# quantumjot/sequitr

Measured on AMD Instinct MI355X. Metric: segmented Mpixels/sec on 512x512 tiles; IoU vs reference, higher is better.
Workload: dtype f32; 1 GPU; U-Net 2-class inference, launches of 32 512x512x1 tiles, fp32 (BASELINE.json configs[1]: filters 16-32-64-128-256, eltwise_mul bridge); logits + uint8 argmax mask; one 32-tile batch per GPU per step; tiles_this_rank=32

## Files before the change

### include/sequitr_hip.h

```cpp
#ifndef SEQUITR_HIP_H
#define SEQUITR_HIP_H

#include <stdint.h>

#ifdef __cplusplus
extern "C" {
#endif

#define SQ_OK 0
#define SQ_EINVAL (-1)
#define SQ_ELAUNCH (-2)
#define SQ_EALIGN (-3)

#define SQ_ACT_NONE 0
#define SQ_ACT_RELU 1
#define SQ_ACT_LEAKY 2

#define SQ_BRIDGE_NONE 0
#define SQ_BRIDGE_ADD 1
#define SQ_BRIDGE_MUL 2
#define SQ_BRIDGE_SUB 3

int sq_version(void);
const char *sq_last_error(void);
// ... 104 lines not shown
int sq_scale_f32(const float *x, float *y, int64_t n, int64_t per_sample, float s, const float *s_per_sample,
                 int one_minus, void *stream);

int sq_act_fwd_f32(const float *x, float *y, int64_t n, int act, void *stream);

int64_t sq_dot_per_sample_workspace_f32(int N);
int sq_dot_per_sample_f32(const float *a, const float *b, float *out, float *workspace, int N, int64_t per_sample,
                          void *stream);

int sq_mbstd_fwd_f32(const float *x, float *out, float *workspace, int N, int64_t per_sample, void *stream);
int64_t sq_mbstd_map_workspace(int groups);
int sq_mbstd_map_fwd_f32(const float *x, float *y, float *workspace, int groups, int n, int64_t per_sample, int cells,
                         void *stream);
int sq_mbstd_map_bwd_f32(const float *x, const float *dy, float *dx, float *workspace, int groups, int n,
                         int64_t per_sample, int cells, void *stream);
int sq_mbstd_map_bwd2_f32(const float *x, const float *dy, const float *v, float *ddy, float *dx2, float *workspace,
                          int groups, int n, int64_t per_sample, int cells, void *stream);
int sq_mbstd_map_fwd_bf16(const void *x, float *y, float *workspace, int groups, int n, int64_t per_sample, int cells, void *stream);
int sq_mbstd_map_bwd_bf16(const void *x, const float *dy, void *dx, float *workspace, int groups, int n, int64_t per_sample,
                          int cells, void *stream);
int sq_mbstd_map_bwd2_bf16(const void *x, const float *dy, const void *v, float *ddy, void *dx2, float *workspace, int groups,
                           int n, int64_t per_sample, int cells, void *stream);
int sq_wgan_losses_fwd_f32(const float *Dz, const float *Dx, const float *gn2, float *out2, int N, void *stream);
int sq_wgan_losses_bwd_f32(const float *Dz, const float *Dx, const float *gn2, const float *g_dloss, const float *g_gloss,
                           float *dDz, float *dDx, float *dgn2, int N, void *stream);

int sq_mosaic_pack_f32(const float *x, float *m, int N, int H, int W, int C, int R, int Cc, void *stream);
int sq_mosaic_unpack_f32(const float *m, float *y, int N, int H, int W, int C, int R, int Cc, void *stream);

int64_t sq_dense_workspace_f32(int M, int K, int N);
int sq_dense_fwd_f32(const float *x, const float *w, const float *bias, float *y, float *workspace, int M, int K, int N,
                     float wscale, int act, void *stream);
int sq_dense_wgrad_f32(const float *x, const float *dy, float *dw, float *db, int M, int K, int N, float scale, int accumulate,
                       void *stream);

int64_t sq_wgrad1x1_small_workspace_f32(int64_t npix, int Ca, int Cb);
int sq_wgrad1x1_small_f32(const float *a, const float *b, float *m, float *workspace, int64_t npix, int Ca, int Cb,
                          void *stream);


int sq_conv2d_concat_nhwc_fwd_f32(const float *xa, const float *xb, const float *w, const float *bias, float *y, int N,
                                  int H, int W, int Ca, int Cout, int K, int act, void *stream);

int sq_conv3x3_pool_fwd_f32(const float *x, const float *w, const float *bias, float *y, float *pooled,
                            int N, int H, int W, int Cin, int Cout, int act, void *stream);

int64_t sq_conv_packed_filter_elems_f32(int K, int Cin, int Cout);
int sq_conv_pack_filter_f32(const float *w, float *wp, int K, int Cin, int Cout, void *stream);
int sq_conv_packed_takes_f32(int N, int H, int W, int Cin, int Cout, int K);
int sq_conv2d_packed_nhwc_fwd_f32(const float *x, const float *w, const float *wp, const float *bias, float *y, int N, int H,
                                  int W, int Cin, int Cout, int K, float wscale, int act, void *stream);
int sq_conv3x3_pool_packed_fwd_f32(const float *x, const float *w, const float *wp, const float *bias, float *y, float *pooled,
                                   int N, int H, int W, int Cin, int Cout, int act, void *stream);

int sq_conv_r32_takes_f32(int N, int H, int W, int Cin, int Cout, int K, int act, int pooled);

int sq_conv3x3_head_fwd_f32(const float *x, const float *w, const float *bias, const float *head_w,
                            const float *head_b, float *logits, uint8_t *mask, int N, int H, int W,
                            int Cin, int head_c, int act, void *stream);

int sq_conv3x3_first_block_fwd_f32(const float *x, const float *w1, const float *b1, const float *w2,
                                   const float *b2, float *y, float *pooled, int N, int H, int W,
                                   void *stream);

int sq_convT_conv3x3_fwd_f32(const float *x_low, const float *wt, const float *bt, const float *skip, int bridge,
                             const float *w, const float *bias, float *y, int N, int H, int W, int act, void *stream);


int64_t sq_conv_packed_weights_elems_bf16(int K, int Cin, int Cout);
int sq_conv_pack_weights_bf16(const float *w, void *wp, int K, int Cin, int Cout, float wscale, int transform,
                              void *stream);
int sq_conv_pack_weights_multi_bf16(const float *base, void *out, const int32_t *table, int n_entries,
                                    int total_items, void *stream);
int sq_conv_pack_weights_multi_scaled_bf16(const float *base, void *out, const int32_t *table, const float *scales,
                                           int n_entries, int total_items, void *stream);

int sq_conv2d_nhwc_fwd_bf16(const void *x, const void *wp, const float *bias, void *y, int N, int H, int W,
                            int Cin, int Cout, int K, int act, void *stream);

int sq_conv2d_nhwc_fwd_mixed_f32(const float *x, const void *wp, const float *bias, float *y, int N, int H, int W,
                                 int Cin, int Cout, int K, int act, void *stream);
int sq_conv2d_nhwc_dgrad_actgate_mixed_f32(const float *dy, const void *wp_t, const float *gate, int act, float *dx, int N,
                                           int H, int W, int Cin, int Cout, int K, void *stream);
int sq_conv2d_nhwc_mixed_mosaic_f32(const float *x, const void *wp, const float *bias, const float *gate, float *y, int Nimg,
                                    int h, int w, int Cin, int Cout, int act, int R, int Cc, void *stream);
int64_t sq_conv2d_nhwc_wgrad_workspace_mixed_f32(int N, int H, int W, int Cin, int Cout, int K);
int sq_conv2d_nhwc_wgrad_mixed_f32(const float *x, const float *dy, float *dw, float *db, float *workspace, int N,
                                   int H, int W, int Cin, int Cout, int K, void *stream);
int sq_conv2d_nhwc_wgrad_scaled_mixed_f32(const float *x, const float *dy, float *dw, float *db, float *workspace, int N,
                                          int H, int W, int Cin, int Cout, int K, float dw_scale, void *stream);
int sq_conv2d_nhwc_wgrad_mixed_mosaic_f32(const float *x, const float *dy, float *dw, float *db, float *workspace, int Nimg,
                                          int h, int w, int Cin, int Cout, int R, int Cc, float dw_scale, void *stream);
int sq_conv2d_nhwc_wgrad_scaled_f32(const float *x, const float *dy, float *dw, float *db, float *workspace, int N, int H,
                                    int W, int Cin, int Cout, int K, float dw_scale, void *stream);

int sq_conv3x3_first_fwd_bf16(const float *x, const float *w, const float *bias, void *y, int N, int H, int W,
                              int Cin, int Cout, int act, void *stream);
int sq_conv3x3_first_fwd_mask_bf16(const float *x, const float *w, const float *bias, void *y, void *mask, int N, int H,
                                   int W, int Cin, int Cout, int act, void *stream);
int sq_conv2d_nhwc_fwd_mask_bf16(const void *x, const void *wp, const float *bias, void *y, void *mask, int N, int H, int W,
                                 int Cin, int Cout, int K, int act, void *stream);
int sq_conv2d_nhwc_dgrad_maskgate_bf16(const void *dy, const void *wp_t, const void *mask, float scale, void *dx, int N,
                                       int H, int W, int Cin, int Cout, int K, void *stream);

int64_t sq_conv2d_nhwc_wgrad_workspace_bf16(int N, int H, int W, int Cin, int Cout, int K);
int sq_conv2d_nhwc_wgrad_bf16(const void *x, const void *dy, float *dw, float *db, float *workspace, int N,
// ... 399 lines not shown
```

### sequitr_amd/_lib.py

```python
import ctypes
import os

_HERE = os.path.dirname(os.path.abspath(__file__))
LIB_PATH = os.path.join(_HERE, "_build", "libsequitr_hip.so")

c_void_p, c_int, c_float, c_int64 = ctypes.c_void_p, ctypes.c_int, ctypes.c_float, ctypes.c_int64


class WgradItem(ctypes.Structure):
    _fields_ = [("x", c_void_p), ("dy", c_void_p), ("dw", c_void_p), ("db", c_void_p),
                ("N", ctypes.c_int32), ("H", ctypes.c_int32), ("W", ctypes.c_int32), ("Cin", ctypes.c_int32),
                ("Cout", ctypes.c_int32), ("K", ctypes.c_int32), ("convT_cout", ctypes.c_int32), ("dw_scale", c_float),
                ("accumulate", ctypes.c_int32), ("mosaic_R", ctypes.c_int32), ("mosaic_Cc", ctypes.c_int32),
                ("reserved", ctypes.c_int32)]

SIGNATURES = {
    "sq_version": (c_int, []),
    "sq_last_error": (ctypes.c_char_p, []),
    "sq_conv2d_nhwc_fwd_f32": (c_int, [c_void_p] * 4 + [c_int] * 6 + [c_float, c_int, c_void_p]),
    "sq_maxpool2x2_fwd_f32": (c_int, [c_void_p] * 2 + [c_int] * 4 + [c_void_p]),
    "sq_avgpool2x2_fwd_f32": (c_int, [c_void_p] * 2 + [c_int] * 4 + [c_void_p]),
    "sq_convT2x2s2_nhwc_fwd_f32": (c_int, [c_void_p] * 5 + [c_int] * 6 + [c_void_p]),
    "sq_bridge_fwd_f32": (c_int, [c_void_p] * 3 + [c_int64, c_int, c_void_p]),
    "sq_conv1x1_argmax_fwd_f32": (c_int, [c_void_p] * 5 + [c_int] * 5 + [c_void_p]),
# ... 102 lines not shown
    "sq_convT_conv3x3_fwd_f32": (c_int, [c_void_p] * 4 + [c_int] + [c_void_p] * 3 + [c_int] * 4 + [c_void_p]),
    "sq_volume_centroids_u8": (c_int, [c_void_p, c_int, c_int, c_int, c_int, c_void_p, c_void_p, c_void_p, c_void_p, c_int,
                                       c_void_p]),
    "sq_mosaic_pack_f32": (c_int, [c_void_p, c_void_p] + [c_int] * 6 + [c_void_p]),
    "sq_mosaic_unpack_f32": (c_int, [c_void_p, c_void_p] + [c_int] * 6 + [c_void_p]),
    "sq_zero_insert2x_f32": (c_int, [c_void_p, c_void_p, c_int, c_int, c_int, c_int, c_void_p]),
    "sq_gather_odd2x_f32": (c_int, [c_void_p, c_void_p, c_int, c_int, c_int, c_int, c_void_p]),
    "sq_bn_workspace_f32": (c_int64, [c_int64, c_int]),
    "sq_bn_stats_f32": (c_int, [c_void_p] * 4 + [c_int64, c_int, c_void_p]),
    "sq_bn_stats_bf16": (c_int, [c_void_p] * 4 + [c_int64, c_int, c_void_p]),
    "sq_bn_fold_f32": (c_int, [c_void_p] * 4 + [c_float, c_void_p, c_void_p, c_int, c_void_p]),
    "sq_bn_update_moving_f32": (c_int, [c_void_p] * 4 + [c_float, c_int64, c_int, c_void_p]),
    "sq_bn_apply_f32": (c_int, [c_void_p] * 4 + [c_int64, c_int, c_int, c_void_p]),
    "sq_bn_apply_bf16": (c_int, [c_void_p] * 4 + [c_int64, c_int, c_int, c_void_p]),
    "sq_bn_bwd_f32": (c_int, [c_void_p] * 3 + [c_int] + [c_void_p] * 3 + [c_float] + [c_void_p] * 4
                      + [c_int64, c_int, c_void_p]),
    "sq_bn_bwd_bf16": (c_int, [c_void_p] * 3 + [c_int] + [c_void_p] * 3 + [c_float] + [c_void_p] * 4
                      + [c_int64, c_int, c_void_p]),
    "sq_adam_step_dev_f32": (c_int, [c_void_p] * 4 + [c_int64] + [c_float] * 4 + [c_void_p, c_float, c_void_p]),
    "sq_adam_advance_dev": (c_int, [c_void_p, c_float, c_float, c_float, c_void_p]),
    "sq_adam_advance_warmup_dev": (c_int, [c_void_p, c_float, c_float, c_float, c_int, c_void_p]),
    "sq_adam_apply_dev_f32": (c_int, [c_void_p] * 4 + [c_int64, c_float, c_float, c_float, c_void_p, c_float, c_void_p]),
    "sq_adam_multi_chunk": (c_int, []),
    "sq_adam_apply_multi_dev_f32": (c_int, [c_void_p, c_int, c_int64, c_float, c_float, c_float, c_void_p, c_float, c_void_p]),
    "sq_pixelnorm_bwd_f32": (c_int, [c_void_p] * 3 + [c_int64, c_int, c_float, c_void_p]),
    "sq_pixelnorm_bwd2_f32": (c_int, [c_void_p] * 5 + [c_int64, c_int, c_float, c_void_p]),
    "sq_pixelnorm_bwd_act_f32": (c_int, [c_void_p] * 3 + [c_int64, c_int, c_float, c_int, c_void_p]),
    "sq_broadcast2x2_act_bwd_f32": (c_int, [c_void_p] * 3 + [c_int] * 4 + [c_float, c_int, c_void_p]),
    "sq_resize_nearest_f32": (c_int, [c_void_p] * 2 + [c_int] * 6 + [c_void_p]),
    "sq_lerp_f32": (c_int, [c_void_p] * 3 + [c_int64, c_int64, c_float, c_void_p, c_void_p]),
    "sq_scale_f32": (c_int, [c_void_p] * 2 + [c_int64, c_int64, c_float, c_void_p, c_int, c_void_p]),
    "sq_act_fwd_f32": (c_int, [c_void_p] * 2 + [c_int64, c_int, c_void_p]),
    "sq_dot_per_sample_workspace_f32": (c_int64, [c_int]),
    "sq_dot_per_sample_f32": (c_int, [c_void_p] * 4 + [c_int, c_int64, c_void_p]),
    "sq_mbstd_fwd_f32": (c_int, [c_void_p] * 3 + [c_int, c_int64, c_void_p]),
    "sq_mbstd_map_workspace": (c_int64, [c_int]),
    "sq_mbstd_map_fwd_f32": (c_int, [c_void_p] * 3 + [c_int, c_int, c_int64, c_int, c_void_p]),
    "sq_mbstd_map_bwd_f32": (c_int, [c_void_p] * 4 + [c_int, c_int, c_int64, c_int, c_void_p]),
    "sq_mbstd_map_bwd2_f32": (c_int, [c_void_p] * 6 + [c_int, c_int, c_int64, c_int, c_void_p]),
    "sq_mbstd_map_fwd_bf16": (c_int, [c_void_p] * 3 + [c_int, c_int, c_int64, c_int, c_void_p]),
    "sq_mbstd_map_bwd_bf16": (c_int, [c_void_p] * 4 + [c_int, c_int, c_int64, c_int, c_void_p]),
    "sq_mbstd_map_bwd2_bf16": (c_int, [c_void_p] * 6 + [c_int, c_int, c_int64, c_int, c_void_p]),
    "sq_wgan_losses_fwd_f32": (c_int, [c_void_p] * 4 + [c_int, c_void_p]),
    "sq_wgan_losses_bwd_f32": (c_int, [c_void_p] * 8 + [c_int, c_void_p]),
    "sq_dense_wgrad_f32": (c_int, [c_void_p] * 4 + [c_int] * 3 + [c_float, c_int, c_void_p]),
    "sq_wgrad1x1_small_workspace_f32": (c_int64, [c_int64, c_int, c_int]),
    "sq_wgrad1x1_small_f32": (c_int, [c_void_p] * 4 + [c_int64, c_int, c_int, c_void_p]),
    "sq_conv2d_concat_nhwc_fwd_f32": (c_int, [c_void_p] * 5 + [c_int] * 7 + [c_void_p]),
    "sq_conv3x3_pool_fwd_f32": (c_int, [c_void_p] * 5 + [c_int] * 6 + [c_void_p]),
    "sq_conv3x3_head_fwd_f32": (c_int, [c_void_p] * 7 + [c_int] * 6 + [c_void_p]),
    "sq_conv_packed_filter_elems_f32": (c_int64, [c_int] * 3),
    "sq_conv_pack_filter_f32": (c_int, [c_void_p] * 2 + [c_int] * 3 + [c_void_p]),
    "sq_conv_packed_takes_f32": (c_int, [c_int] * 6),
    "sq_conv_r32_takes_f32": (c_int, [c_int] * 8),
    "sq_conv2d_packed_nhwc_fwd_f32": (c_int, [c_void_p] * 5 + [c_int] * 6 + [c_float, c_int, c_void_p]),
    "sq_conv3x3_pool_packed_fwd_f32": (c_int, [c_void_p] * 6 + [c_int] * 6 + [c_void_p]),
    "sq_conv3x3_first_block_fwd_f32": (c_int, [c_void_p] * 7 + [c_int] * 3 + [c_void_p]),
    "sq_conv_packed_weights_elems_bf16": (c_int64, [c_int] * 3),
    "sq_conv_pack_weights_bf16": (c_int, [c_void_p] * 2 + [c_int] * 3 + [c_float, c_int, c_void_p]),
    "sq_conv2d_nhwc_fwd_bf16": (c_int, [c_void_p] * 4 + [c_int] * 7 + [c_void_p]),
    "sq_conv2d_nhwc_fwd_mixed_f32": (c_int, [c_void_p] * 4 + [c_int] * 7 + [c_void_p]),
    "sq_conv2d_nhwc_wgrad_workspace_mixed_f32": (c_int64, [c_int] * 6),
    "sq_conv2d_nhwc_wgrad_mixed_f32": (c_int, [c_void_p] * 5 + [c_int] * 6 + [c_void_p]),
    "sq_conv2d_nhwc_wgrad_scaled_mixed_f32": (c_int, [c_void_p] * 5 + [c_int] * 6 + [c_float, c_void_p]),
    "sq_conv2d_nhwc_wgrad_scaled_f32": (c_int, [c_void_p] * 5 + [c_int] * 6 + [c_float, c_void_p]),
    "sq_conv3x3_first_fwd_bf16": (c_int, [c_void_p] * 4 + [c_int] * 6 + [c_void_p]),
    "sq_conv2d_nhwc_wgrad_workspace_bf16": (c_int64, [c_int] * 6),
    "sq_conv2d_nhwc_wgrad_bf16": (c_int, [c_void_p] * 5 + [c_int] * 6 + [c_void_p]),
    "sq_convT2x2s2_wgrad_bf16": (c_int, [c_void_p] * 5 + [c_int] * 5 + [c_void_p]),
    "sq_cast_f32_to_bf16": (c_int, [c_void_p] * 2 + [c_int64, c_void_p]),
    "sq_cast_bf16_to_f32": (c_int, [c_void_p] * 2 + [c_int64, c_void_p]),
    "sq_head_concat_fwd_bf16": (c_int, [c_void_p] * 3 + [c_int64, c_int, c_void_p]),
    "sq_head_concat_bwd_bf16": (c_int, [c_void_p] * 3 + [c_int64, c_int, c_void_p]),
    "sq_maxpool2x2_fwd_bf16": (c_int, [c_void_p] * 2 + [c_int] * 4 + [c_void_p]),
    "sq_maxpool2x2_bwd_bf16": (c_int, [c_void_p] * 3 + [c_int] * 4 + [c_void_p]),
    "sq_conv_pack_weights_multi_bf16": (c_int, [c_void_p, c_void_p, c_void_p, c_int, c_int, c_void_p]),
    "sq_conv_pack_weights_multi_scaled_bf16": (c_int, [c_void_p] * 4 + [c_int, c_int, c_void_p]),
    "sq_conv2d_nhwc_fwd_dropout_bf16": (c_int, [c_void_p] * 4 + [c_int] * 7 + [c_float, ctypes.c_uint32, c_void_p, c_void_p]),
    "sq_conv3x3_first_fwd_mask_bf16": (c_int, [c_void_p] * 5 + [c_int] * 6 + [c_void_p]),
    "sq_conv2d_nhwc_fwd_mask_bf16": (c_int, [c_void_p] * 5 + [c_int] * 7 + [c_void_p]),
    "sq_conv2d_nhwc_dgrad_maskgate_bf16": (c_int, [c_void_p] * 3 + [c_float, c_void_p] + [c_int] * 6 + [c_void_p]),
    "sq_conv2d_nhwc_wgrad_mixed_mosaic_f32": (c_int, [c_void_p] * 5 + [c_int] * 7 + [c_float, c_void_p]),
    "sq_conv2d_nhwc_mixed_mosaic_f32": (c_int, [c_void_p] * 5 + [c_int] * 8 + [c_void_p]),
    "sq_conv2d_nhwc_dgrad_actgate_mixed_f32": (c_int, [c_void_p] * 3 + [c_int, c_void_p] + [c_int] * 6 + [c_void_p]),
    "sq_conv2d_nhwc_fwd_dropout_pool_bf16": (c_int, [c_void_p] * 5 + [c_int] * 7 + [c_float, ctypes.c_uint32, c_void_p, c_void_p]),
    "sq_conv3x3_first_block_dropout_pool_bf16": (c_int, [c_void_p] * 9 + [c_int] * 3 + [c_float, ctypes.c_uint32, c_void_p, c_void_p]),
    "sq_relu_scale_bwd_bf16": (c_int, [c_void_p] * 3 + [c_int64, c_float, c_void_p]),
    "sq_bridge_bwd_s2d_bf16": (c_int, [c_void_p] * 5 + [c_int] * 5 + [c_void_p]),
    "sq_maxpool2x2_bwd_add_bf16": (c_int, [c_void_p] * 4 + [c_int] * 4 + [c_void_p]),
    "sq_maxpool2x2_bwd_add_gate_bf16": (c_int, [c_void_p] * 4 + [c_int] * 4 + [c_float, c_void_p]),
    "sq_conv2d_nhwc_dgrad_gate_bf16": (c_int, [c_void_p] * 3 + [c_float, c_void_p] + [c_int] * 6 + [c_void_p]),
    "sq_conv2d_nhwc_dgrad_junction_bf16": (c_int, [c_void_p] * 6 + [c_int] * 7 + [c_void_p]),
    "sq_conv1x1_head_bwd_gate_bf16": (c_int, [c_void_p] * 7 + [c_int64, c_int, c_int, c_float, c_void_p]),
    "sq_conv1x1_head_wce_fwd_bf16": (c_int, [c_void_p] * 7 + [c_int64, c_int, c_int, c_void_p]),
    "sq_conv1x1_head_wce_bwd_bf16": (c_int, [c_void_p] * 10 + [c_int64, c_int, c_int, c_float, c_void_p]),
    "sq_conv1x1_head_wce_bwd_loss_bf16": (c_int, [c_void_p] * 12 + [c_int64, c_int, c_int, c_float, c_void_p]),
    "sq_act_dropout_bwd_bf16": (c_int, [c_void_p] * 4 + [c_int64, c_float, c_int, c_void_p]),
    "sq_conv2d_nhwc_dgrad_relu_bf16": (c_int, [c_void_p] * 4 + [c_int] * 6 + [c_void_p]),
    "sq_pixelnorm_fwd_bf16": (c_int, [c_void_p] * 2 + [c_int64, c_int, c_float, c_void_p]),
    "sq_pixelnorm_bwd_bf16": (c_int, [c_void_p] * 3 + [c_int64, c_int, c_float, c_int, c_void_p]),
    "sq_pixelnorm_bwd2_bf16": (c_int, [c_void_p] * 5 + [c_int64, c_int, c_float, c_void_p]),
    "sq_sumpool2x2_bf16": (c_int, [c_void_p] * 2 + [c_int] * 4 + [c_float, c_void_p]),
    "sq_broadcast2x2_bf16": (c_int, [c_void_p] * 2 + [c_int] * 4 + [c_float, c_void_p]),
    "sq_broadcast2x2_act_bwd_bf16": (c_int, [c_void_p] * 3 + [c_int] * 4 + [c_float, c_int, c_void_p]),
    "sq_act_fwd_bf16": (c_int, [c_void_p] * 2 + [c_int64, c_int, c_void_p]),
    "sq_conv1x1_smallin_fwd_bf16": (c_int, [c_void_p] * 4 + [c_int64, c_int, c_int, c_float, c_int, c_void_p]),
# ... 72 lines not shown
```

### sequitr_amd/csrc/sq_conv_f32_packed.hip

```cpp
#include <stdlib.h>
#include <type_traits>
#include "sq_common.h"
#include "sq_conv_epi.h"

#ifndef SQ_PK_RING
#define SQ_PK_RING 4
#endif
#ifndef SQ_PK_OCC
#define SQ_PK_OCC 2
#endif
#ifndef SQ_PK_WRITE_AT
#define SQ_PK_WRITE_AT 22
#endif

namespace {

constexpr int TH = 16, TW = 16, BN = 64, KC = 16, NR = BN / 16;
constexpr int HALO_W = TW + 2, HALO_H = TH + 2, HP = HALO_W * HALO_H;
constexpr int PS = KC + 2;
constexpr int XS_FLOATS = HP * PS;
constexpr int QPP = KC / 4, XITEMS = HP * QPP, XSLOTS = (XITEMS + 255) / 256;
constexpr int NSTEP = 9 * (KC / 4);
constexpr int RING = SQ_PK_RING;
constexpr int STEP_BYTES = 64 * 16, ITEM_BYTES = NSTEP * STEP_BYTES;
constexpr int LDS_BYTES = (2 * XS_FLOATS + 64 * 4) * 4;
constexpr int OCC = SQ_PK_OCC;
static_assert(SQ_PK_OCC != 2 || sq_v2_occ(BN, KC, false) == 2, "the default walks the unpacked form's grid");
static_assert(NSTEP % RING == 0 && RING >= 2 && RING <= 6, "the ring slot of a step must not depend on the item");
static_assert(SQ_PK_WRITE_AT + XSLOTS <= NSTEP, "the halo writes must fit the item's steps");
static_assert((XS_FLOATS * 4) % 16 == 0, "second halo buffer must start 16-B aligned");

__global__ __launch_bounds__(256) void pack_filter_f32_kernel(const float *__restrict__ w, float4 *__restrict__ wp,
                                                              int Cin, int Cout, int total) {
    const int e = blockIdx.x * 256 + threadIdx.x;
    if (e >= total) return;
    const int lane = e & 63, li = lane & 15, kk = lane >> 4;
    int t = e >> 6;
    const int s = t & 3;
    t >>= 2;
    const int tap = t % 9;
    t /= 9;
    const int nchunk = Cin / KC, c = t % nchunk, cb = t / nchunk;
    const float *src = w + (size_t)(tap * Cin + c * KC + 4 * s + kk) * Cout + cb * BN + li;
    wp[e] = make_float4(src[0], src[16], src[32], src[48]);
}

__global__ __launch_bounds__(256, OCC) void conv_mfma_f32_packed_kernel(
    const float *__restrict__ x, const float *__restrict__ wp, const float *__restrict__ bias, float *__restrict__ y,
    int N, int H, int W, int Cin, int Cout, int act, int tiles_x, int tiles_y, int ntiles, float *__restrict__ pooled) {
    extern __shared__ __attribute__((aligned(16))) float smem[];
    const int tid = threadIdx.x, lane = tid & 63, wv = tid >> 6;
    __builtin_assume(tid < 256);
    const int li = lane & 15, kk = lane >> 4;
    const int n0 = blockIdx.y * BN;
    const int vb = (int)sq_xcd_remap(blockIdx.x, gridDim.x);
    const int tstride = (int)gridDim.x;
    const int t_begin = vb;
    if (t_begin >= ntiles) return;
    const int t_count = (ntiles - vb + tstride - 1) / tstride;
    const int nchunk = Cin / KC;
    const int nitems = t_count * nchunk;

    const __amdgpu_buffer_rsrc_t xrsrc = __builtin_amdgcn_make_buffer_rsrc(
        const_cast<float *>(x), 0, (int)((size_t)N * H * W * Cin * 4), 0x00020000);
    const __amdgpu_buffer_rsrc_t wrsrc = __builtin_amdgcn_make_buffer_rsrc(
        const_cast<float *>(wp), 0, 9 * Cin * Cout * 4, 0x00020000);
    const __amdgpu_buffer_rsrc_t yrsrc = __builtin_amdgcn_make_buffer_rsrc(y, 0, (int)((size_t)N * H * W * Cout * 4), 0x00020000);
    constexpr unsigned OOB = 0x80000000u;

    int xrel[XSLOTS], xpy[XSLOTS], xpx[XSLOTS];
#pragma unroll
    for (int sl = 0; sl < XSLOTS; ++sl) {
        const int idx = tid + sl * 256;
        const int pix = idx / QPP, q = idx % QPP;
        xpy[sl] = idx < XITEMS ? pix / HALO_W : (1 << 24);
        xpx[sl] = pix % HALO_W;
        xrel[sl] = idx < XITEMS ? ((pix / HALO_W * W + xpx[sl]) * Cin + q * 4) * 4 : (int)OOB;
    }
    float4 xr[XSLOTS];
    auto issue = [&](int tx, int ty, int n, int cc, bool live) {
        const int x0 = tx * TW - 1, y0 = ty * TH - 1;
        const int base = (((n * H + y0) * W + x0) * Cin + cc) * 4;
        const unsigned Hl = live ? (unsigned)H : 0u;
#pragma unroll
        for (int sl = 0; sl < XSLOTS; ++sl) {
            const bool inb = (unsigned)(y0 + xpy[sl]) < Hl && (unsigned)(x0 + xpx[sl]) < (unsigned)W;
            const unsigned off = inb ? (unsigned)(base + xrel[sl]) : OOB;
            const auto v = __builtin_amdgcn_raw_buffer_load_b128(xrsrc, off, 0, 0);
            xr[sl] = *reinterpret_cast<const float4 *>(&v);
        }
    };
    float *const dump = smem + 2 * XS_FLOATS + lane * 4;
    auto put_slot = [&](float *xs, int sl) {
        const int idx = tid + sl * 256;
        const int pix = idx / QPP, q = idx % QPP;
        float *d = idx < XITEMS ? xs + pix * PS + q * 4 : dump;
        *reinterpret_cast<float2 *>(d) = make_float2(xr[sl].x, xr[sl].y);
        *reinterpret_cast<float2 *>(d + 2) = make_float2(xr[sl].z, xr[sl].w);
    };

    const int a_lane = lane * 16;
    auto load_a = [&](int item_off, int st) {
        const auto v = __builtin_amdgcn_raw_buffer_load_b128(wrsrc, a_lane, item_off + st * STEP_BYTES, 0);
        return *reinterpret_cast<const float4 *>(&v);
    };
    const int xb_off = ((4 * wv) * HALO_W + li) * PS + kk;
    auto load_b = [&](const float *xs, int st, float (&b)[4]) {
        const int tap = st / 4, s = st % 4;
        const int ky = tap / 3, kx = tap % 3;
#pragma unroll
        for (int r = 0; r < 4; ++r) b[r] = xs[xb_off + ((r + ky) * HALO_W + kx) * PS + s * 4];
    };

    const float slope = act == SQ_ACT_LEAKY ? 0.2f : 1.0f;
    const bool is_relu = act == SQ_ACT_RELU;
    auto actk = [&](float v, auto fastc) {
        if constexpr (decltype(fastc)::value) return __builtin_fmaxf(v, 0.0f);
        else {
            const float neg = is_relu ? 0.0f : v * slope;
            return v > 0.0f ? v : neg;
        }
    };
    float4 bvr[NR];
#pragma unroll
    for (int nb = 0; nb < NR; ++nb)
        bvr[nb] = bias ? *reinterpret_cast<const float4 *>(bias + n0 + nb * 16 + 4 * kk) : make_float4(0.f, 0.f, 0.f, 0.f);
    const int fast_lane = (((4 * wv) * W + li) * Cout + 4 * kk) * 4;

    f32x4 acc[4][NR];
    auto epilogue = [&](int tx, int ty, int n, auto fastc) {
        constexpr bool FAST = decltype(fastc)::value;
        auto actf = [&](float v) { return actk(v, fastc); };
        const int gx = tx * TW + li;
#pragma unroll
        for (int nb = 0; nb < NR; ++nb) {
            const int co = n0 + nb * 16 + 4 * kk;
            const float4 bv = bvr[nb];
            f32x4 o[4];
#pragma unroll
            for (int r = 0; r < 4; ++r) {
                const int gy = ty * TH + 4 * wv + r;
                o[r][0] = actf(bias ? acc[r][nb][0] + bv.x : acc[r][nb][0]);
                o[r][1] = actf(bias ? acc[r][nb][1] + bv.y : acc[r][nb][1]);
                o[r][2] = actf(bias ? acc[r][nb][2] + bv.z : acc[r][nb][2]);
                o[r][3] = actf(bias ? acc[r][nb][3] + bv.w : acc[r][nb][3]);
                unsigned off;
                if constexpr (FAST) {
                    off = (unsigned)(fast_lane + nb * 64) + (unsigned)((((n * H + ty * TH + r) * W + tx * TW) * Cout + n0) * 4);
                } else {
                    const bool ok = gy < H && gx < W;
                    off = ok ? (unsigned)((((n * H + gy) * W + gx) * Cout + co) * 4) : OOB;
                }
                __builtin_amdgcn_raw_buffer_store_b128(
                    *reinterpret_cast<__attribute__((__vector_size__(4 * sizeof(unsigned)))) unsigned *>(&o[r]), yrsrc, off, 0, 0);
                acc[r][nb] = (f32x4){0.f, 0.f, 0.f, 0.f};
            }
            if (pooled) {
#pragma unroll
                for (int pr = 0; pr < 2; ++pr) {
                    float mp[4];
#pragma unroll
                    for (int j = 0; j < 4; ++j) {
                        const float a = o[2 * pr][j], b = o[2 * pr + 1][j];
                        const float v = b > a ? b : a;
                        const float u = __shfl_xor(v, 1);
                        mp[j] = u > v ? u : v;
                    }
                    const int py = (ty * TH + 4 * wv) / 2 + pr, px = gx >> 1;
                    if ((li & 1) == 0 && py < (H >> 1) && px < (W >> 1))
                        *reinterpret_cast<float4 *>(pooled + ((size_t)(n * (H >> 1) + py) * (W >> 1) + px) * Cout + co) =
                            make_float4(mp[0], mp[1], mp[2], mp[3]);
                }
            }
        }
    };

    const int per_image = tiles_x * tiles_y;
    const int s_n = tstride / per_image, s_y = (tstride % per_image) / tiles_x, s_x = (tstride % per_image) % tiles_x;
    int ctx = t_begin % tiles_x, cty = (t_begin / tiles_x) % tiles_y, cn = t_begin / per_image;
    int ntx = ctx + s_x, nty = cty, nn = cn;
    if (ntx >= tiles_x) { ntx -= tiles_x; nty += 1; }
    nty += s_y;
    if (nty >= tiles_y) { nty -= tiles_y; nn += 1; }
    nn += s_n;

    const int cb_off = blockIdx.y * nchunk * ITEM_BYTES;
    issue(ctx, cty, cn, 0, true);
    float4 ar[RING];
#pragma unroll
    for (int j = 0; j < RING; ++j) ar[j] = load_a(cb_off, j);
#pragma unroll
    for (int sl = 0; sl < XSLOTS; ++sl) put_slot(smem, sl);
#pragma unroll
    for (int r = 0; r < 4; ++r)
#pragma unroll
        for (int nb = 0; nb < NR; ++nb) acc[r][nb] = (f32x4){0.f, 0.f, 0.f, 0.f};
    __syncthreads();

    int chunk = 0;
    for (int it = 0; it < nitems; ++it) {
        const float *xs = smem + (it & 1) * XS_FLOATS;
        float *xo = smem + ((it & 1) ^ 1) * XS_FLOATS;
        int nchk = chunk + 1;
        const bool same = nchk != nchunk;
        if (!same) nchk = 0;
        const bool has_next = it + 1 < nitems;
        issue(same ? ctx : ntx, same ? cty : nty, same ? cn : nn, nchk * KC, has_next);
        const int item_off = cb_off + chunk * ITEM_BYTES, next_off = cb_off + nchk * ITEM_BYTES;
        {
            float b0[4], b1[4];
            load_b(xs, 0, b0);
            __builtin_amdgcn_s_setprio(0);
#pragma unroll
            for (int st = 0; st < NSTEP; ++st) {
                float (&bc)[4] = (st & 1) ? b1 : b0;
                float (&bn)[4] = (st & 1) ? b0 : b1;
                const float4 a = ar[st % RING];
                if (st + 1 < NSTEP) load_b(xs, st + 1, bn);
                if (st >= SQ_PK_WRITE_AT && st < SQ_PK_WRITE_AT + XSLOTS) put_slot(xo, st - SQ_PK_WRITE_AT);
                __builtin_amdgcn_sched_barrier(0);
                const float av[NR] = {a.x, a.y, a.z, a.w};
#pragma unroll
                for (int r = 0; r < 4; ++r)
#pragma unroll
                    for (int nb = 0; nb < NR; ++nb)
                        acc[r][nb] = __builtin_amdgcn_mfma_f32_16x16x4f32(av[nb], bc[r], acc[r][nb], 0, 0, 0);
                ar[st % RING] = st + RING < NSTEP ? load_a(item_off, st + RING) : load_a(next_off, st + RING - NSTEP);
                __builtin_amdgcn_sched_barrier(0);
            }
            __builtin_amdgcn_s_setprio(3);
        }
        __syncthreads();
        if (!same) {
            const bool fast = is_relu && cty * TH + TH <= H && ctx * TW + TW <= W;
            if (fast) epilogue(ctx, cty, cn, std::integral_constant<bool, true>{});
            else epilogue(ctx, cty, cn, std::integral_constant<bool, false>{});
            ctx = ntx; cty = nty; cn = nn;
            ntx += s_x;
            if (ntx >= tiles_x) { ntx -= tiles_x; nty += 1; }
            nty += s_y;
            if (nty >= tiles_y) { nty -= tiles_y; nn += 1; }
            nn += s_n;
        }
        chunk = nchk;
    }
}

bool packed_switch_on() {
    const char *e = getenv("SQ_CONV_PACKED");
    return !(e && e[0] == '0');
}

bool pack_eligible(int K, int Cin, int Cout) { return K == 3 && Cin > 0 && Cin % KC == 0 && Cout > 0 && Cout % BN == 0; }

}

extern "C" int64_t sq_conv_packed_filter_elems_f32(int K, int Cin, int Cout) {
    return pack_eligible(K, Cin, Cout) ? (int64_t)9 * Cin * Cout : -1;
}

extern "C" int sq_conv_pack_filter_f32(const float *w, float *wp, int K, int Cin, int Cout, void *stream) {
    SQ_REQUIRE(w && wp, "sq_conv_pack_filter_f32: null pointer");
    SQ_REQUIRE(pack_eligible(K, Cin, Cout), "sq_conv_pack_filter_f32: unsupported K=%d Cin=%d Cout=%d (3x3, Cin %% 16 == 0, Cout %% 64 == 0)",
               K, Cin, Cout);
    SQ_REQUIRE((int64_t)9 * Cin * Cout * 4 < ((int64_t)1 << 31), "sq_conv_pack_filter_f32: the pack must be < 2 GiB");
    SQ_REQUIRE_ALIGNED(w); SQ_REQUIRE_ALIGNED(wp);
    const int total = 9 * Cin * Cout / 4;
    hipLaunchKernelGGL(pack_filter_f32_kernel, dim3((total + 255) / 256), dim3(256), 0, reinterpret_cast<hipStream_t>(stream),
                       w, reinterpret_cast<float4 *>(wp), Cin, Cout, total);
    return sq_check_launch("sq_conv_pack_filter_f32");
}

extern "C" int sq_conv_packed_takes_f32(int N, int H, int W, int Cin, int Cout, int K) {
    if (N <= 0 || H <= 0 || W <= 0 || !pack_eligible(K, Cin, Cout) || !packed_switch_on()) return 0;
    if ((size_t)N * H * W * (size_t)(Cin > Cout ? Cin : Cout) * 4 >= ((size_t)1 << 31)) return 0;
    const int64_t ntiles = (int64_t)((W + TW - 1) / TW) * ((H + TH - 1) / TH) * N;
    return sq_plan_f32_bn(ntiles, Cout) == 64 ? 1 : 0;
}

static int sq_conv_packed_launch(const float *x, const float *wp, const float *bias, float *y, float *pooled, int N, int H, int W,
                          int Cin, int Cout, int act, hipStream_t st) {
    static bool attr_set = false;
    if (!attr_set) {
        if (hipFuncSetAttribute(reinterpret_cast<const void *>(conv_mfma_f32_packed_kernel),
                                hipFuncAttributeMaxDynamicSharedMemorySize, LDS_BYTES) != hipSuccess) {
            sq_set_error("conv_mfma_f32_packed: cannot reserve %d bytes of LDS", LDS_BYTES);
            return SQ_ELAUNCH;
        }
        attr_set = true;
    }
    const int tiles_x = (W + TW - 1) / TW, tiles_y = (H + TH - 1) / TH;
    const int ntiles = tiles_x * tiles_y * N;
    const int gy = Cout / BN;
    int tpb;
    const int gx = sq_plan_v2_grid(ntiles, gy, OCC, &tpb);
    hipLaunchKernelGGL(conv_mfma_f32_packed_kernel, dim3(gx, gy), dim3(256), LDS_BYTES, st, x, wp, bias, y, N, H, W, Cin, Cout,
                       act, tiles_x, tiles_y, ntiles, pooled);
    return sq_check_launch("sq_conv2d_packed_nhwc_fwd_f32");
}

namespace {
int packed_args_ok(const char *who, const float *x, const float *wp, const float *bias, const float *y, const float *pooled,
                   int N, int H, int W, int Cin, int Cout, int act) {
    SQ_REQUIRE(x && y, "%s: null tensor pointer", who);
    SQ_REQUIRE(act >= SQ_ACT_NONE && act <= SQ_ACT_LEAKY, "%s: bad activation %d", who, act);
    SQ_REQUIRE_ALIGNED(x); SQ_REQUIRE_ALIGNED(wp); SQ_REQUIRE_ALIGNED(y);
    if (bias) SQ_REQUIRE_ALIGNED(bias);
    if (pooled) SQ_REQUIRE_ALIGNED(pooled);
    return SQ_OK;
}
}

extern "C" int sq_conv2d_packed_nhwc_fwd_f32(const float *x, const float *w, const float *wp, const float *bias, float *y,
                                             int N, int H, int W, int Cin, int Cout, int K, float wscale, int act, void *stream) {
    static const bool impl1 = [] { const char *e = getenv("SQ_CONV_IMPL"); return e && e[0] == '1'; }();
    if (!wp || wscale != 1.0f || impl1 || !sq_conv_packed_takes_f32(N, H, W, Cin, Cout, K))
        return sq_conv2d_nhwc_fwd_f32(x, w, bias, y, N, H, W, Cin, Cout, K, wscale, act, stream);
    const int rc = packed_args_ok("sq_conv2d_packed_nhwc_fwd_f32", x, wp, bias, y, nullptr, N, H, W, Cin, Cout, act);
    if (rc != SQ_OK) return rc;
    return sq_conv_packed_launch(x, wp, bias, y, nullptr, N, H, W, Cin, Cout, act, reinterpret_cast<hipStream_t>(stream));
}

extern "C" int sq_conv3x3_pool_packed_fwd_f32(const float *x, const float *w, const float *wp, const float *bias, float *y,
                                              float *pooled, int N, int H, int W, int Cin, int Cout, int act, void *stream) {
    if (!wp || !pooled || H % 2 || W % 2 || !sq_conv_packed_takes_f32(N, H, W, Cin, Cout, 3))
        return sq_conv3x3_pool_fwd_f32(x, w, bias, y, pooled, N, H, W, Cin, Cout, act, stream);
    const int rc = packed_args_ok("sq_conv3x3_pool_packed_fwd_f32", x, wp, bias, y, pooled, N, H, W, Cin, Cout, act);
    if (rc != SQ_OK) return rc;
    return sq_conv_packed_launch(x, wp, bias, y, pooled, N, H, W, Cin, Cout, act, reinterpret_cast<hipStream_t>(stream));
}
```

### sequitr_amd/ops.py

```python
import os

import torch

from . import _lib

ACT = {None: 0, "none": 0, "relu": 1, "leaky": 2}
BRIDGE = {None: 0, "none": 0, "eltwise_add": 1, "eltwise_mul": 2, "eltwise_sub": 3}


def _stream():
    return torch.cuda.current_stream().cuda_stream


def _chk(t, name, dtype=torch.float32, ndim=None):
    if not isinstance(t, torch.Tensor):
        raise TypeError("%s must be a torch.Tensor" % name)
    if not t.is_cuda:
        raise _lib.SequitrHipError("%s must live in GPU memory (no CPU fallback exists)" % name)
    if t.dtype != dtype:
        raise TypeError("%s must be %s, got %s" % (name, dtype, t.dtype))
    if not t.is_contiguous():
        raise ValueError("%s must be contiguous (NHWC)" % name)
    if ndim is not None and t.dim() != ndim:
        raise ValueError("%s must have %d dims, got %s" % (name, ndim, tuple(t.shape)))
# ... 144 lines not shown
                _ptr(self.flat), _ptr(self.out), _ptr(self.table), _ptr(self.scales), self.n, self.total, _stream()),
                "sq_conv_pack_weights_multi_scaled_bf16")
        self.fresh = True

    def lookup(self, w, K, Cin, Cout, wscale, transform):
        base = w._base if w._base is not None else w
        e = self.views.get((id(base), bool(transform)))
        if e is None or not self.fresh:
            return None
        d0, n, ws, k, ci, co = e
        if (k, ci, co) != (K, Cin, Cout) or ws != float(wscale):
            return None
        return self.out[d0:d0 + n]


class FilterPackF32(object):

    def __init__(self, w):
        _chk(w, "w", ndim=4)
        K, K2, Cin, Cout = w.shape
        n = _lib.load().sq_conv_packed_filter_elems_f32(K, Cin, Cout) if K == K2 else -1
        if n <= 0:
            raise ValueError("no f32 filter pack for a %s filter (3x3, Cin %% 16 == 0, Cout %% 64 == 0)" % (tuple(w.shape),))
        self.w = w
        self.wp = torch.empty((n,), dtype=torch.float32, device=w.device)
        self.epoch = None
        self.repack()

    def repack(self):
        K, _, Cin, Cout = self.w.shape
        self.epoch = invalidation_epoch()
        _lib.check(_lib.load().sq_conv_pack_filter_f32(_ptr(self.w), _ptr(self.wp), K, Cin, Cout, _stream()),
                   "sq_conv_pack_filter_f32")

    def current(self, w):
        if w is not self.w:
            raise ValueError("pack= belongs to another filter tensor than the call's w")
        if self.epoch != invalidation_epoch():
            self.repack()
        return self.wp


def pack_filter(w):
    if w.dim() != 4 or w.shape[0] != w.shape[1] or w.dtype != torch.float32:
        return None
    if _lib.load().sq_conv_packed_filter_elems_f32(w.shape[0], w.shape[2], w.shape[3]) <= 0:
        return None
    return FilterPackF32(w)


def conv_packed_takes(x_shape, w_shape):
    N, H, W, Cin = x_shape
    return bool(_lib.load().sq_conv_packed_takes_f32(N, H, W, Cin, w_shape[3], w_shape[0])) and w_shape[2] == Cin


def conv_r32_takes(x_shape, w_shape, act="relu", pooled=False):
    N, H, W, Cin = x_shape
    return bool(_lib.load().sq_conv_r32_takes_f32(N, H, W, Cin, w_shape[3], w_shape[0], ACT[act], 1 if pooled else 0)) \
        and w_shape[2] == Cin


def _packed_filter(w, K, Cin, Cout, wscale, transform):
    for plan in list(_PLANS):
        wp = plan.lookup(w, K, Cin, Cout, wscale, transform)
        if wp is not None:
            return wp
    cacheable = w.is_leaf and w.requires_grad
    key = (w.data_ptr(), K, Cin, Cout, float(wscale), bool(transform))
    if cacheable and key in _PACKS:
        return _PACKS[key][1]
    lib = _lib.load()
    n = lib.sq_conv_packed_weights_elems_bf16(K, Cin, Cout)
    wp = torch.empty((n,), dtype=torch.bfloat16, device=w.device)
    _lib.check(lib.sq_conv_pack_weights_bf16(_ptr(w), _ptr(wp), K, Cin, Cout, float(wscale), 1 if transform else 0,
                                            _stream()), "sq_conv_pack_weights_bf16")
    if cacheable:
        _PACKS[key] = (w, wp)
    return wp


def _conv2d_mixed(x, w, bias, act, wscale, y, transform):
    N, H, W, Cin = x.shape
    K, Cout = w.shape[0], (w.shape[2] if transform else w.shape[3])
    lib = _lib.load()
    wp = _packed_filter(w, K, Cin, Cout, wscale, transform)
    _lib.check(lib.sq_conv2d_nhwc_fwd_mixed_f32(_ptr(x), _ptr(wp), _ptr(bias), _ptr(y), N, H, W, Cin, Cout, K, ACT[act],
                                               _stream()), "sq_conv2d_nhwc_fwd_mixed_f32")
    return y


def dense(x, w, bias=None, act=None, wscale=1.0):
    _chk(x, "x", ndim=2), _chk(w, "w", ndim=2)
    M, K = x.shape
    N = w.shape[1]
    if w.shape[0] != K:
        raise ValueError("dense: weight %s does not match %d inputs" % (tuple(w.shape), K))
    if bias is not None:
        _chk(bias, "bias")
    lib = _lib.load()
    ws = _workspace(lib.sq_dense_workspace_f32(M, K, N), x.device)
    y = torch.empty((M, N), dtype=torch.float32, device=x.device)
    _lib.check(lib.sq_dense_fwd_f32(_ptr(x), _ptr(w), _ptr(bias), _ptr(y), _ptr(ws), M, K, N, float(wscale), ACT[act],
                                   _stream()), "sq_dense_fwd_f32")
    return y


# ... 1305 lines not shown
```

Measured before the change: 1729 Mpixels/s.

## Overlap packed conv epilogue stores with the last K-chunk's MFMA steps

Adds a templated closing form of the packed fp32 MFMA 3x3 conv kernel. The last input-channel chunk of each tile is processed one output row at a time, and the bias, activation, stores and optional 2x2 max-pool of finished rows are interleaved into the MFMA steps of the following rows. Bias is staged in LDS for this path. The goal is to hide the epilogue's global stores behind matrix work instead of running a separate serial epilogue after the final chunk. In exchange the per-row grouping issues narrower B loads, adds register pressure and code size, and is enabled by default for Cin >= 32.

```diff
diff --git a/include/sequitr_hip.h b/include/sequitr_hip.h
--- a/include/sequitr_hip.h
+++ b/include/sequitr_hip.h
@@ -180,6 +180,10 @@
                                   int W, int Cin, int Cout, int K, float wscale, int act, void *stream);
 int sq_conv3x3_pool_packed_fwd_f32(const float *x, const float *w, const float *wp, const float *bias, float *y, float *pooled,
                                    int N, int H, int W, int Cin, int Cout, int act, void *stream);
+
+int sq_conv_packed_close_takes_f32(int N, int H, int W, int Cin, int Cout, int K);
+int sq_conv_packed_form_f32(const float *x, const float *wp, const float *bias, float *y, float *pooled, int N, int H, int W,
+                            int Cin, int Cout, int act, int close, void *stream);
 
 int sq_conv_r32_takes_f32(int N, int H, int W, int Cin, int Cout, int K, int act, int pooled);
 
diff --git a/sequitr_amd/_lib.py b/sequitr_amd/_lib.py
--- a/sequitr_amd/_lib.py
+++ b/sequitr_amd/_lib.py
@@ -178,6 +178,8 @@
     "sq_conv_packed_filter_elems_f32": (c_int64, [c_int] * 3),
     "sq_conv_pack_filter_f32": (c_int, [c_void_p] * 2 + [c_int] * 3 + [c_void_p]),
     "sq_conv_packed_takes_f32": (c_int, [c_int] * 6),
+    "sq_conv_packed_close_takes_f32": (c_int, [c_int] * 6),
+    "sq_conv_packed_form_f32": (c_int, [c_void_p] * 5 + [c_int] * 7 + [c_void_p]),
     "sq_conv_r32_takes_f32": (c_int, [c_int] * 8),
     "sq_conv2d_packed_nhwc_fwd_f32": (c_int, [c_void_p] * 5 + [c_int] * 6 + [c_float, c_int, c_void_p]),
     "sq_conv3x3_pool_packed_fwd_f32": (c_int, [c_void_p] * 6 + [c_int] * 6 + [c_void_p]),
diff --git a/sequitr_amd/csrc/sq_conv_f32_packed.hip b/sequitr_amd/csrc/sq_conv_f32_packed.hip
--- a/sequitr_amd/csrc/sq_conv_f32_packed.hip
+++ b/sequitr_amd/csrc/sq_conv_f32_packed.hip
@@ -13,6 +13,16 @@
 #define SQ_PK_WRITE_AT 22
 #endif
 
+#ifndef SQ_PK_CLOSE_ROWS
+#define SQ_PK_CLOSE_ROWS 1
+#endif
+#ifndef SQ_PK_CLOSE_STORE_AT
+#define SQ_PK_CLOSE_STORE_AT 1
+#endif
+#ifndef SQ_PK_CLOSE_STORE_GAP
+#define SQ_PK_CLOSE_STORE_GAP 2
+#endif
+
 namespace {
 
 constexpr int TH = 16, TW = 16, BN = 64, KC = 16, NR = BN / 16;
@@ -24,11 +34,17 @@
 constexpr int RING = SQ_PK_RING;
 constexpr int STEP_BYTES = 64 * 16, ITEM_BYTES = NSTEP * STEP_BYTES;
 constexpr int LDS_BYTES = (2 * XS_FLOATS + 64 * 4) * 4;
+constexpr int LDS_BYTES_CLOSE = LDS_BYTES + BN * 4;
 constexpr int OCC = SQ_PK_OCC;
 static_assert(SQ_PK_OCC != 2 || sq_v2_occ(BN, KC, false) == 2, "the default walks the unpacked form's grid");
-static_assert(NSTEP % RING == 0 && RING >= 2 && RING <= 6, "the ring slot of a step must not depend on the item");
+static_assert(NSTEP % RING == 0 && RING >= 2 && RING <= 12, "the ring slot of a step must not depend on the item");
 static_assert(SQ_PK_WRITE_AT + XSLOTS <= NSTEP, "the halo writes must fit the item's steps");
 static_assert((XS_FLOATS * 4) % 16 == 0, "second halo buffer must start 16-B aligned");
+constexpr int RG = SQ_PK_CLOSE_ROWS;
+static_assert(RG == 1 || (RG == 2 && SQ_PK_CLOSE_STORE_GAP == 0), "the closing item goes by rows, or by row pairs with a pair's stores "
+              "at one step (spread over steps the pair form is not fully unrolled and the accumulators go to scratch)");
+static_assert(SQ_PK_CLOSE_STORE_GAP >= 0 && SQ_PK_CLOSE_STORE_AT >= 0 && SQ_PK_CLOSE_STORE_AT + (RG * 4 - 1) * SQ_PK_CLOSE_STORE_GAP < NSTEP,
+              "a group's stores must fit the following group's steps");
 
 __global__ __launch_bounds__(256) void pack_filter_f32_kernel(const float *__restrict__ w, float4 *__restrict__ wp,
                                                               int Cin, int Cout, int total) {
@@ -45,6 +61,7 @@
     wp[e] = make_float4(src[0], src[16], src[32], src[48]);
 }
 
+template <bool CLOSE>
 __global__ __launch_bounds__(256, OCC) void conv_mfma_f32_packed_kernel(
     const float *__restrict__ x, const float *__restrict__ wp, const float *__restrict__ bias, float *__restrict__ y,
     int N, int H, int W, int Cin, int Cout, int act, int tiles_x, int tiles_y, int ntiles, float *__restrict__ pooled) {
@@ -112,6 +129,12 @@
         for (int r = 0; r < 4; ++r) b[r] = xs[xb_off + ((r + ky) * HALO_W + kx) * PS + s * 4];
     };
 
+    auto load_b1 = [&](const float *xs, int r, int st) {
+        const int tap = st / 4, s = st % 4;
+        const int ky = tap / 3, kx = tap % 3;
+        return xs[xb_off + ((r + ky) * HALO_W + kx) * PS + s * 4];
+    };
+
     const float slope = act == SQ_ACT_LEAKY ? 0.2f : 1.0f;
     const bool is_relu = act == SQ_ACT_RELU;
     auto actk = [&](float v, auto fastc) {
@@ -121,6 +144,8 @@
             return v > 0.0f ? v : neg;
         }
     };
+    float *const bsm = smem + 2 * XS_FLOATS + 64 * 4;
+    if (CLOSE && tid < BN) bsm[tid] = bias ? bias[n0 + tid] : 0.0f;
     float4 bvr[NR];
 #pragma unroll
     for (int nb = 0; nb < NR; ++nb)
@@ -175,6 +200,46 @@
         }
     };
 
+    auto close_quad = [&](int r, int nb, int tx, int ty, int n, auto fastc) {
+        constexpr bool FAST = decltype(fastc)::value;
+        const float4 bv = *reinterpret_cast<const float4 *>(bsm + nb * 16 + 4 * kk);
+        f32x4 &o = acc[r][nb];
+        o[0] = actk(bias ? o[0] + bv.x : o[0], fastc);
+        o[1] = actk(bias ? o[1] + bv.y : o[1], fastc);
+        o[2] = actk(bias ? o[2] + bv.z : o[2], fastc);
+        o[3] = actk(bias ? o[3] + bv.w : o[3], fastc);
+        unsigned off;
+        if constexpr (FAST) {
+            off = (unsigned)(fast_lane + nb * 64) + (unsigned)((((n * H + ty * TH + r) * W + tx * TW) * Cout + n0) * 4);
+        } else {
+            const int gx = tx * TW + li, gy = ty * TH + 4 * wv + r, co = n0 + nb * 16 + 4 * kk;
+            const bool ok = gy < H && gx < W;
+            off = ok ? (unsigned)((((n * H + gy) * W + gx) * Cout + co) * 4) : OOB;
+        }
+        __builtin_amdgcn_raw_buffer_store_b128(
+            *reinterpret_cast<__attribute__((__vector_size__(4 * sizeof(unsigned)))) unsigned *>(&o), yrsrc, off, 0, 0);
+    };
+    auto close_pool = [&](int pr, int nb, int tx, int ty, int n) {
+        float mp[4];
+#pragma unroll
+        for (int j = 0; j < 4; ++j) {
+            const float a = acc[2 * pr][nb][j], b = acc[2 * pr + 1][nb][j];
+            const float v = b > a ? b : a;
+            const float u = __shfl_xor(v, 1);
+            mp[j] = u > v ? u : v;
+        }
+        const int gx = tx * TW + li, co = n0 + nb * 16 + 4 * kk;
+        const int py = (ty * TH + 4 * wv) / 2 + pr, px = gx >> 1;
+        if ((li & 1) == 0 && py < (H >> 1) && px < (W >> 1))
+            *reinterpret_cast<float4 *>(pooled + ((size_t)(n * (H >> 1) + py) * (W >> 1) + px) * Cout + co) =
+                make_float4(mp[0], mp[1], mp[2], mp[3]);
+    };
+    auto close_emit = [&](int r, int nb, int tx, int ty, int n, bool fast) {
+        if (fast) close_quad(r, nb, tx, ty, n, std::integral_constant<bool, true>{});
+        else close_quad(r, nb, tx, ty, n, std::integral_constant<bool, false>{});
+        if ((r & 1) && pooled) close_pool(r >> 1, nb, tx, ty, n);
+    };
+
     const int per_image = tiles_x * tiles_y;
     const int s_n = tstride / per_image, s_y = (tstride % per_image) / tiles_x, s_x = (tstride % per_image) % tiles_x;
     int ctx = t_begin % tiles_x, cty = (t_begin / tiles_x) % tiles_y, cn = t_begin / per_image;
@@ -197,8 +262,107 @@
         for (int nb = 0; nb < NR; ++nb) acc[r][nb] = (f32x4){0.f, 0.f, 0.f, 0.f};
     __syncthreads();
 
+    int it = 0;
+    auto mul_item = [&](const float *xs, float *xo, int item_off, int next_off) {
+        float b0[4], b1[4];
+        load_b(xs, 0, b0);
+        __builtin_amdgcn_s_setprio(0);
+#pragma unroll
+        for (int st = 0; st < NSTEP; ++st) {
+            float (&bc)[4] = (st & 1) ? b1 : b0;
+            float (&bn)[4] = (st & 1) ? b0 : b1;
+            const float4 a = ar[st % RING];
+            if (st + 1 < NSTEP) load_b(xs, st + 1, bn);
+            if (st >= SQ_PK_WRITE_AT && st < SQ_PK_WRITE_AT + XSLOTS) put_slot(xo, st - SQ_PK_WRITE_AT);
+            __builtin_amdgcn_sched_barrier(0);
+            const float av[NR] = {a.x, a.y, a.z, a.w};
+#pragma unroll
+            for (int r = 0; r < 4; ++r)
+#pragma unroll
+                for (int nb = 0; nb < NR; ++nb)
+                    acc[r][nb] = __builtin_amdgcn_mfma_f32_16x16x4f32(av[nb], bc[r], acc[r][nb], 0, 0, 0);
+            ar[st % RING] = st + RING < NSTEP ? load_a(item_off, st + RING) : load_a(next_off, st + RING - NSTEP);
+            __builtin_amdgcn_sched_barrier(0);
+        }
+        __builtin_amdgcn_s_setprio(3);
+    };
+    auto mul_closing = [&](const float *xs, float *xo, int item_off, int next_off, bool fast) {
+        float b0[RG], b1[RG];
+#pragma unroll
+        for (int j = 0; j < RG; ++j) b0[j] = load_b1(xs, j, 0);
+        __builtin_amdgcn_s_setprio(0);
+#pragma unroll
+        for (int rg = 0; rg < 4; rg += RG) {
+#pragma unroll
+            for (int st = 0; st < NSTEP; ++st) {
+                const int g = (rg / RG) * NSTEP + st;
+                float (&bc)[RG] = (g & 1) ? b1 : b0;
+                float (&bn)[RG] = (g & 1) ? b0 : b1;
+                const float4 a = ar[g % RING];
+                if (g + 1 < 4 / RG * NSTEP) {
+#pragma unroll
+                    for (int j = 0; j < RG; ++j) bn[j] = load_b1(xs, (g + 1) / NSTEP * RG + j, (g + 1) % NSTEP);
+                }
+                if (rg == 4 - RG && st >= SQ_PK_WRITE_AT && st < SQ_PK_WRITE_AT + XSLOTS) put_slot(xo, st - SQ_PK_WRITE_AT);
+                __builtin_amdgcn_sched_barrier(0);
+                const float av[NR] = {a.x, a.y, a.z, a.w};
+#pragma unroll
+                for (int j = 0; j < RG; ++j)
+#pragma unroll
+                    for (int nb = 0; nb < NR; ++nb)
+                        acc[rg + j][nb] = __builtin_amdgcn_mfma_f32_16x16x4f32(av[nb], bc[j], acc[rg + j][nb], 0, 0, 0);
+                ar[st % RING] = st + RING < NSTEP ? load_a(item_off, st + RING)
+                                : rg < 4 - RG     ? load_a(item_off, st + RING - NSTEP)
+                                                  : load_a(next_off, st + RING - NSTEP);
+                if (rg > 0) {
+#pragma unroll
+                    for (int j = 0; j < RG; ++j)
+#pragma unroll
+                        for (int nb = 0; nb < NR; ++nb)
+                            if (st == SQ_PK_CLOSE_STORE_AT + (j * NR + nb) * SQ_PK_CLOSE_STORE_GAP) close_emit(rg - RG + j, nb, ctx, cty, cn, fast);
+                }
+                __builtin_amdgcn_sched_barrier(0);
+            }
+        }
+        __builtin_amdgcn_s_setprio(3);
+    };
+    auto advance = [&]() {
+        ctx = ntx; cty = nty; cn = nn;
+        ntx += s_x;
+        if (ntx >= tiles_x) { ntx -= tiles_x; nty += 1; }
+        nty += s_y;
+        if (nty >= tiles_y) { nty -= tiles_y; nn += 1; }
+        nn += s_n;
+    };
+
+    if constexpr (CLOSE) {
+        for (int t = 0; t < t_count; ++t) {
+            for (int chunk = 0; chunk + 1 < nchunk; ++chunk, ++it) {
+                issue(ctx, cty, cn, (chunk + 1) * KC, true);
+                mul_item(smem + (it & 1) * XS_FLOATS, smem + ((it & 1) ^ 1) * XS_FLOATS, cb_off + chunk * ITEM_BYTES,
+                         cb_off + (chunk + 1) * ITEM_BYTES);
+                __syncthreads();
+            }
+            issue(ntx, nty, nn, 0, t + 1 < t_count);
+            const bool fast = is_relu && cty * TH + TH <= H && ctx * TW + TW <= W;
+            mul_closing(smem + (it & 1) * XS_FLOATS, smem + ((it & 1) ^ 1) * XS_FLOATS, cb_off + (nchunk - 1) * ITEM_BYTES, cb_off, fast);
+            __syncthreads();
+#pragma unroll
+            for (int j = 0; j < RG; ++j)
+#pragma unroll
+                for (int nb = 0; nb < NR; ++nb) close_emit(4 - RG + j, nb, ctx, cty, cn, fast);
+#pragma unroll
+            for (int r = 0; r < 4; ++r)
+#pragma unroll
+                for (int nb = 0; nb < NR; ++nb) acc[r][nb] = (f32x4){0.f, 0.f, 0.f, 0.f};
+            advance();
+            ++it;
+        }
+        return;
+    }
+
     int chunk = 0;
-    for (int it = 0; it < nitems; ++it) {
+    for (; it < nitems; ++it) {
         const float *xs = smem + (it & 1) * XS_FLOATS;
         float *xo = smem + ((it & 1) ^ 1) * XS_FLOATS;
         int nchk = chunk + 1;
@@ -207,40 +371,13 @@
         const bool has_next = it + 1 < nitems;
         issue(same ? ctx : ntx, same ? cty : nty, same ? cn : nn, nchk * KC, has_next);
         const int item_off = cb_off + chunk * ITEM_BYTES, next_off = cb_off + nchk * ITEM_BYTES;
-        {
-            float b0[4], b1[4];
-            load_b(xs, 0, b0);
-            __builtin_amdgcn_s_setprio(0);
-#pragma unroll
-            for (int st = 0; st < NSTEP; ++st) {
-                float (&bc)[4] = (st & 1) ? b1 : b0;
-                float (&bn)[4] = (st & 1) ? b0 : b1;
-                const float4 a = ar[st % RING];
-                if (st + 1 < NSTEP) load_b(xs, st + 1, bn);
-                if (st >= SQ_PK_WRITE_AT && st < SQ_PK_WRITE_AT + XSLOTS) put_slot(xo, st - SQ_PK_WRITE_AT);
-                __builtin_amdgcn_sched_barrier(0);
-                const float av[NR] = {a.x, a.y, a.z, a.w};
-#pragma unroll
-                for (int r = 0; r < 4; ++r)
-#pragma unroll
-                    for (int nb = 0; nb < NR; ++nb)
-                        acc[r][nb] = __builtin_amdgcn_mfma_f32_16x16x4f32(av[nb], bc[r], acc[r][nb], 0, 0, 0);
-                ar[st % RING] = st + RING < NSTEP ? load_a(item_off, st + RING) : load_a(next_off, st + RING - NSTEP);
-                __builtin_amdgcn_sched_barrier(0);
-            }
-            __builtin_amdgcn_s_setprio(3);
-        }
+        mul_item(xs, xo, item_off, next_off);
         __syncthreads();
         if (!same) {
             const bool fast = is_relu && cty * TH + TH <= H && ctx * TW + TW <= W;
             if (fast) epilogue(ctx, cty, cn, std::integral_constant<bool, true>{});
             else epilogue(ctx, cty, cn, std::integral_constant<bool, false>{});
-            ctx = ntx; cty = nty; cn = nn;
-            ntx += s_x;
-            if (ntx >= tiles_x) { ntx -= tiles_x; nty += 1; }
-            nty += s_y;
-            if (nty >= tiles_y) { nty -= tiles_y; nn += 1; }
-            nn += s_n;
+            advance();
         }
         chunk = nchk;
     }
@@ -250,6 +387,13 @@
     const char *e = getenv("SQ_CONV_PACKED");
     return !(e && e[0] == '0');
 }
+
+bool close_switch_on() {
+    const char *e = getenv("SQ_CONV_PACKED_CLOSE");
+    return !(e && e[0] == '0');
+}
+
+bool close_shape_rule(int Cin) { return Cin >= 2 * KC; }
 
 bool pack_eligible(int K, int Cin, int Cout) { return K == 3 && Cin > 0 && Cin % KC == 0 && Cout > 0 && Cout % BN == 0; }
 
@@ -278,13 +422,20 @@
     return sq_plan_f32_bn(ntiles, Cout) == 64 ? 1 : 0;
 }
 
-static int sq_conv_packed_launch(const float *x, const float *wp, const float *bias, float *y, float *pooled, int N, int H, int W,
-                          int Cin, int Cout, int act, hipStream_t st) {
+extern "C" int sq_conv_packed_close_takes_f32(int N, int H, int W, int Cin, int Cout, int K) {
+    if (!sq_conv_packed_takes_f32(N, H, W, Cin, Cout, K) || !close_switch_on()) return 0;
+    return close_shape_rule(Cin) ? 1 : 0;
+}
+
+template <bool CLOSE>
+static int sq_conv_packed_launch_form(const float *x, const float *wp, const float *bias, float *y, float *pooled, int N, int H, int W,
+                                      int Cin, int Cout, int act, hipStream_t st) {
+    constexpr int LDS = CLOSE ? LDS_BYTES_CLOSE : LDS_BYTES;
     static bool attr_set = false;
     if (!attr_set) {
-        if (hipFuncSetAttribute(reinterpret_cast<const void *>(conv_mfma_f32_packed_kernel),
-                                hipFuncAttributeMaxDynamicSharedMemorySize, LDS_BYTES) != hipSuccess) {
-            sq_set_error("conv_mfma_f32_packed: cannot reserve %d bytes of LDS", LDS_BYTES);
+        if (hipFuncSetAttribute(reinterpret_cast<const void *>(conv_mfma_f32_packed_kernel<CLOSE>),
+                                hipFuncAttributeMaxDynamicSharedMemorySize, LDS) != hipSuccess) {
+            sq_set_error("conv_mfma_f32_packed: cannot reserve %d bytes of LDS", LDS);
             return SQ_ELAUNCH;
         }
         attr_set = true;
@@ -294,9 +445,16 @@
     const int gy = Cout / BN;
     int tpb;
     const int gx = sq_plan_v2_grid(ntiles, gy, OCC, &tpb);
-    hipLaunchKernelGGL(conv_mfma_f32_packed_kernel, dim3(gx, gy), dim3(256), LDS_BYTES, st, x, wp, bias, y, N, H, W, Cin, Cout,
+    hipLaunchKernelGGL(conv_mfma_f32_packed_kernel<CLOSE>, dim3(gx, gy), dim3(256), LDS, st, x, wp, bias, y, N, H, W, Cin, Cout,
                        act, tiles_x, tiles_y, ntiles, pooled);
     return sq_check_launch("sq_conv2d_packed_nhwc_fwd_f32");
+}
+
+static int sq_conv_packed_launch(const float *x, const float *wp, const float *bias, float *y, float *pooled, int N, int H, int W,
+                                 int Cin, int Cout, int act, hipStream_t st) {
+    if (sq_conv_packed_close_takes_f32(N, H, W, Cin, Cout, 3))
+        return sq_conv_packed_launch_form<true>(x, wp, bias, y, pooled, N, H, W, Cin, Cout, act, st);
+    return sq_conv_packed_launch_form<false>(x, wp, bias, y, pooled, N, H, W, Cin, Cout, act, st);
 }
 
 namespace {
@@ -329,3 +487,16 @@
     if (rc != SQ_OK) return rc;
     return sq_conv_packed_launch(x, wp, bias, y, pooled, N, H, W, Cin, Cout, act, reinterpret_cast<hipStream_t>(stream));
 }
+
+extern "C" int sq_conv_packed_form_f32(const float *x, const float *wp, const float *bias, float *y, float *pooled, int N, int H,
+                                       int W, int Cin, int Cout, int act, int close, void *stream) {
+    SQ_REQUIRE(N > 0 && H > 0 && W > 0 && pack_eligible(3, Cin, Cout), "sq_conv_packed_form_f32: unsupported N=%d H=%d W=%d Cin=%d Cout=%d",
+               N, H, W, Cin, Cout);
+    SQ_REQUIRE((size_t)N * H * W * (size_t)(Cin > Cout ? Cin : Cout) * 4 < ((size_t)1 << 31), "sq_conv_packed_form_f32: tensors must be < 2 GiB");
+    SQ_REQUIRE(wp, "sq_conv_packed_form_f32: null pack");
+    SQ_REQUIRE(!pooled || (H % 2 == 0 && W % 2 == 0), "sq_conv_packed_form_f32: the pooled output needs even H and W");
+    const int rc = packed_args_ok("sq_conv_packed_form_f32", x, wp, bias, y, pooled, N, H, W, Cin, Cout, act);
+    if (rc != SQ_OK) return rc;
+    if (close) return sq_conv_packed_launch_form<true>(x, wp, bias, y, pooled, N, H, W, Cin, Cout, act, reinterpret_cast<hipStream_t>(stream));
+    return sq_conv_packed_launch_form<false>(x, wp, bias, y, pooled, N, H, W, Cin, Cout, act, reinterpret_cast<hipStream_t>(stream));
+}
diff --git a/sequitr_amd/ops.py b/sequitr_amd/ops.py
--- a/sequitr_amd/ops.py
+++ b/sequitr_amd/ops.py
@@ -220,6 +220,11 @@
 def conv_packed_takes(x_shape, w_shape):
     N, H, W, Cin = x_shape
     return bool(_lib.load().sq_conv_packed_takes_f32(N, H, W, Cin, w_shape[3], w_shape[0])) and w_shape[2] == Cin
+
+
+def conv_packed_close_takes(x_shape, w_shape):
+    N, H, W, Cin = x_shape
+    return bool(_lib.load().sq_conv_packed_close_takes_f32(N, H, W, Cin, w_shape[3], w_shape[0])) and w_shape[2] == Cin
 
 
 def conv_r32_takes(x_shape, w_shape, act="relu", pooled=False):
```

New measurement: 1741 Mpixels/s, median of 6. Within noise of the previous version (+0.7%).
